# distributed-lab/bp-pp

Hardware: AMD Instinct MI355X
Metric: u64 range-proof batch verifies/sec (higher is better)
Workload: dtype u32; 1 GPU; batch verify ONE fixed batch of 1048576 independent u64 range proofs (BASELINE configs[2]; all resident on one GPU), exact per-proof mode, shared generators, inputs resident in HBM, 1/1024 proofs corrupted, one 4-byte reject-count all-reduce per step; proofs_per_gpu=1048576, fb_window_bits=523, fb_window_bits_hi=0, fb_hi_bases=0, fb_window_bits_chosen_by=the library, from the HBM free at context creation, label=u64 range proof, parallelism=single, full=False

## Files before the change

bp_pp_amd/csrc/straus_core.h:

```cpp
#pragma once
#include "verify_ws.h"

namespace bppp {

struct straus_scalar { u32 kp[8]; u32 top; };
HD void straus_recode(straus_scalar& r, const sc& k) {
    u64 c = 0;
#pragma unroll
    for (int i = 0; i < 8; i++) { c += (u64)k.v[i] + 0x88888888u; r.kp[i] = (u32)c; c >>= 32; }
    r.top = (u32)c;
}
HD void straus_build_table(pt_slot* tbl, const apt& P) {
    pt cur;
    pt_set_identity(cur);
    tbl[0].p = cur;
    pt_from_affine(cur, P);
    tbl[1].p = cur;
    const bool pid = apt_is_identity(P);
#pragma nounroll
    for (int e = 2; e <= 8; e++) {
        pt src = tbl[(e & 1) ? e - 1 : e / 2].p;
        pt d;
        if (e & 1) pt_madd(d, src, P, pid);
        else pt_dbl(d, src);
        pt_normalize(d);
        tbl[e].p = d;
    }
}
HD void straus_msm(pt& out, const pt_slot* tbl, const straus_scalar* rs, int m) {
    pt acc;
    pt_set_identity(acc);
#pragma nounroll
    for (int j = 0; j < m; j++) {
        pt q = tbl[j * BPPP_STRAUS_ENTRIES + (rs[j].top ? 1 : 0)].p;
        pt_add(acc, acc, q);
    }
#pragma nounroll
    for (int i = 63; i >= 0; i--) {
#pragma nounroll
        for (int d = 0; d < 4; d++) pt_dbl(acc, acc);
#pragma nounroll
        for (int j = 0; j < m; j++) {
            u32 limb = 0;
#pragma unroll
            for (int l = 0; l < 8; l++) limb = (l == (i >> 3)) ? rs[j].kp[l] : limb;
            int dg = (int)((limb >> ((i & 7) * 4)) & 15) - 8;
            int mag = dg < 0 ? -dg : dg;
            pt q = tbl[j * BPPP_STRAUS_ENTRIES + mag].p;
            fe ny;
            fe_neg_m<1>(ny, q.Y);
            fe_cmov(q.Y, dg < 0, ny);
            pt_add(acc, acc, q);
        }
    }
    out = acc;
}

struct glv_split { u32 k1[5], k2[5]; bool neg1, neg2; };
HD void glv_round_shift384(sc& c, const sc& k, const u32 g[8]) {
    u32 t[16];
    mul256(t, k.v, g);
    u32 cy = (t[11] >> 31) & 1u;
#pragma unroll
    for (int i = 0; i < 4; i++) c.v[i] = addc(t[12 + i], 0u, cy);
#pragma unroll
    for (int i = 4; i < 8; i++) c.v[i] = 0;
}
HD bool glv_abs(u32 out[5], const sc& r) {
    bool neg = ((r.v[5] | r.v[6] | r.v[7]) != 0) | (r.v[4] > 1u);
    sc m;
    sc_neg(m, r);
#pragma unroll
    for (int i = 0; i < 5; i++) out[i] = neg ? m.v[i] : r.v[i];
    return neg;
}
HD void glv_decompose(glv_split& out, const sc& k) {
    const u32 G1[8] = {0x45DBB031u, 0xE893209Au, 0x71E8CA7Fu, 0x3DAA8A14u, 0x9284EB15u, 0xE86C90E4u, 0xA7D46BCDu, 0x3086D221u};
    const u32 G2[8] = {0x8AC47F71u, 0x1571B4AEu, 0x9DF506C6u, 0x221208ACu, 0x0ABFE4C4u, 0x6F547FA9u, 0x010E8828u, 0xE4437ED6u};
    const sc MB1 = {{0x0ABFE4C3u, 0x6F547FA9u, 0x010E8828u, 0xE4437ED6u, 0x00000000u, 0x00000000u, 0x00000000u, 0x00000000u}};
    const sc MB2 = {{0x3DB1562Cu, 0xD765CDA8u, 0x0774346Du, 0x8A280AC5u, 0xFFFFFFFEu, 0xFFFFFFFFu, 0xFFFFFFFFu, 0xFFFFFFFFu}};
    const sc LAM = {{0x1B23BD72u, 0xDF02967Cu, 0x20816678u, 0x122E22EAu, 0x8812645Au, 0xA5261C02u, 0xC05C30E0u, 0x5363AD4Cu}};
    sc c1, c2, r1, r2, t;
    glv_round_shift384(c1, k, G1);
    glv_round_shift384(c2, k, G2);
    sc_mul(c1, c1, MB1);
    sc_mul(c2, c2, MB2);
    sc_add(r2, c1, c2);
    sc_mul(t, r2, LAM);
    sc_sub(r1, k, t);
    out.neg1 = glv_abs(out.k1, r1);
    out.neg2 = glv_abs(out.k2, r2);
    u32 c = 0;
#pragma unroll
    for (int i = 0; i < 5; i++) out.k1[i] = addc(out.k1[i], i < 4 ? 0x88888888u : 0x8u, c);
    c = 0;
#pragma unroll
    for (int i = 0; i < 5; i++) out.k2[i] = addc(out.k2[i], i < 4 ? 0x88888888u : 0x8u, c);
}
HD u32 limb5_at(const u32 v[5], int idx) {
    u32 r = 0;
#pragma unroll
    for (int l = 0; l < 5; l++) r = (l == idx) ? v[l] : r;
    return r;
}
HD void straus_msm_glv(pt& out, const pt_slot* tbl, const glv_split* sp, int m) {
    const u32 BETA_W[8] = {0x719501EEu, 0xC1396C28u, 0x12F58995u, 0x9CF04975u, 0xAC3434E9u, 0x6E64479Eu, 0x657C0710u, 0x7AE96A2Bu};
    fe BETA;
    fe_from_w8(BETA, BETA_W);
    pt acc;
    pt_set_identity(acc);
#pragma nounroll
    for (int i = 32; i >= 0; i--) {
        if (i != 32) {
#pragma nounroll
            for (int d = 0; d < 4; d++) pt_dbl(acc, acc);
        }
#pragma nounroll
        for (int j = 0; j < m; j++) {
#pragma nounroll
            for (int h = 0; h < 2; h++) {
                const u32* kp = h ? sp[j].k2 : sp[j].k1;
                bool sneg = h ? sp[j].neg2 : sp[j].neg1;
                int dg = (int)((limb5_at(kp, i >> 3) >> ((i & 7) * 4)) & 15) - 8;
                int mag = dg < 0 ? -dg : dg;
                pt q = tbl[j * BPPP_STRAUS_ENTRIES + mag].p;
                fe bx, ny;
                fe_mul(bx, q.X, BETA);
                fe_cmov(q.X, h != 0, bx);
                fe_neg_m<1>(ny, q.Y);
                fe_cmov(q.Y, (dg < 0) != sneg, ny);
                pt_add(acc, acc, q);
            }
        }
    }
    out = acc;
}

#define BPPP_VPOINTS 13
#define BPPP_ATAB_PER_PROOF (BPPP_VPOINTS * 16)
HD void ws_st_fe(u32* base, size_t N, size_t t, int slot, const fe& a) {
#pragma unroll
    for (int i = 0; i < 10; i++) base[(size_t)(slot * 10 + i) * N + t] = a.v[i];
}
HD void ws_ld_fe(fe& a, const u32* base, size_t N, size_t t, int slot, int mag) {
#pragma unroll
    for (int i = 0; i < 10; i++) a.v[i] = base[(size_t)(slot * 10 + i) * N + t];
    FE_SETMAG(a, mag);
    (void)mag;
}
template <int G>
HD void fe_batch_inv_lane(const u32* in, u32* out, size_t N, size_t i) {
    const size_t L = (N + G - 1) / G;
    fe z[G], pre[G], run, inv, one;
    bool zero[G];
    fe_set_u32(one, 1);
    run = one;
#pragma unroll
    for (int j = 0; j < G; j++) {
        const size_t t = i + (size_t)j * L;
        z[j] = one;
        zero[j] = true;
        if (t < N) {
            ws_ld_fe(z[j], in, N, t, 0, 2);
            zero[j] = fe_is_zero(z[j]);
            if (zero[j]) z[j] = one;
        }
        pre[j] = run;
        fe_mul(run, run, z[j]);
    }
    fe_inv(inv, run);
#pragma unroll
    for (int j = G - 1; j >= 0; j--) {
        const size_t t = i + (size_t)j * L;
        fe o;
        fe_mul(o, inv, pre[j]);
        fe_mul(inv, inv, z[j]);
        if (zero[j]) fe_set_u32(o, 0);
        if (t < N) ws_st_fe(out, N, t, 0, o);
    }
}
HD void glv_beta(fe& b) {
    const u32 BETA_W[8] = {0x719501EEu, 0xC1396C28u, 0x12F58995u, 0x9CF04975u, 0xAC3434E9u, 0x6E64479Eu, 0x657C0710u, 0x7AE96A2Bu};
    fe_from_w8(b, BETA_W);
}
struct atab_ref {
    apt_packed* p;
    size_t s;
    HD apt_packed& operator[](int i) const { return p[(size_t)i * s]; }
    HD atab_ref operator+(int k) const { atab_ref r = {p + (size_t)k * s, s}; return r; }
};
HD atab_ref atab_of(apt_packed* atab, size_t N, size_t t, int entries_per_instance = 13 * 16) {
    (void)entries_per_instance;
    atab_ref r = {atab + t, N};
    return r;
}
HD void atab_store(atab_ref tb, int e, const apt& a, const fe& beta, bool identity) {
    apt_packed k;
    fe_to_w8(k.x, a.x);
    fe_to_w8(k.y, a.y);
    if (identity) {
#pragma unroll
        for (int i = 0; i < 8; i++) k.x[i] = k.y[i] = 0;
    }
    tb[e - 1] = k;
    (void)beta;
}
#define BPPP_TSCR_FE (5 * BPPP_VPOINTS)
struct aff_src { fe x, y; };
HD void aff_ld(aff_src& r, atab_ref tb, int e) {
    const apt_packed k = tb[e - 1];
    fe_from_w8(r.x, k.x);
    fe_from_w8(r.y, k.y);
}
HD void aff_den_dbl(fe& d, const aff_src& a, bool pid, const fe& one) { fe_add(d, a.y, a.y); fe_cmov(d, pid, one); }
HD void aff_den_add(fe& d, const aff_src& a, const aff_src& b, bool pid, const fe& one) { fe_sub_m<1>(d, a.x, b.x); fe_cmov(d, pid, one); }
HD void aff_dbl(apt& r, const aff_src& a, const fe& dinv) {
    fe num, lam, t;
    fe_sqr(num, a.x);
    fe_mul_small(num, num, 3);
    fe_mul(lam, num, dinv);
    fe_sqr(r.x, lam);
    fe_add(t, a.x, a.x);
    fe_sub_m<2>(r.x, r.x, t);
    fe_sub_m<4>(t, a.x, r.x);
    fe_mul(t, lam, t);
    fe_sub_m<1>(r.y, t, a.y);
}
HD void aff_add(apt& r, const aff_src& a, const aff_src& b, const fe& dinv) {
    fe num, lam, t;
    fe_sub_m<1>(num, a.y, b.y);
    fe_mul(lam, num, dinv);
    fe_sqr(r.x, lam);
    fe_sub_m<1>(r.x, r.x, a.x);
    fe_sub_m<1>(r.x, r.x, b.x);
    fe_sub_m<5>(t, a.x, r.x);
    fe_mul(t, lam, t);
    fe_sub_m<1>(r.y, t, a.y);
}
HD void aff_take(aff_src& r, const apt& a) {
    fe_mul_small(r.x, a.x, 1);
    fe_mul_small(r.y, a.y, 1);
}
HD void aff_push(u32* tscr, size_t N, size_t t, int slot, fe& run, const fe& den) {
    ws_st_fe(tscr, N, t, slot, run);
    fe_mul(run, run, den);
}
HD void aff_pop(fe& dinv, const u32* tscr, size_t N, size_t t, int slot, fe& inv, const fe& den) {
    fe pre;
    ws_ld_fe(pre, tscr, N, t, slot, 1);
    fe_mul(dinv, inv, pre);
    fe_mul(inv, inv, den);
}
HD void aff_push_block(u32* tscr, size_t N, size_t t, int slot, fe& run, const fe& block_product) {
    ws_st_fe(tscr, N, t, slot, run);
    fe_mul(run, run, block_product);
}
HD void aff_pop_block(fe di[4], const fe d[4], const u32* tscr, size_t N, size_t t, int slot, fe& inv) {
    fe t01, t23, B, pre, q;
    fe_mul(t01, d[0], d[1]);
    fe_mul(t23, d[2], d[3]);
    fe_mul(B, t01, t23);
    ws_ld_fe(pre, tscr, N, t, slot, 1);
    fe_mul(q, inv, pre);
    fe_mul(inv, inv, B);
    fe_mul(B, q, t23);
    fe_mul(q, q, t01);
    fe_mul(di[0], B, d[1]);
    fe_mul(di[1], B, d[0]);
    fe_mul(di[2], q, d[3]);
    fe_mul(di[3], q, d[2]);
}
#define BPPP_TSCR_PER_POINT 5
HD void affine_tables_pass_a(const atab_ref tab, u32* tscr, const u32* pts, size_t N, size_t t, const int NP, fe& run) {
    const int L2 = NP, L4 = 3 * NP;
    (void)L2; (void)L4;
    fe beta, one, d, dinv;
    fe_set_u32(one, 1);
    glv_beta(beta);
    (void)d; (void)dinv;
    fe_set_u32(run, 1);
#pragma nounroll
    for (int p = 0; p < NP; p++) {
        apt P;
        ws_ld_apt(P, pts, N, t, p);
        const bool pid = apt_is_identity(P);
        atab_store(tab + p * 16, 1, P, beta, pid);
        aff_src a = {P.x, P.y};
        aff_den_dbl(d, a, pid, one);
        aff_push(tscr, N, t, p, run, d);
    }
}
HD void affine_tables_pass_b(const atab_ref tab, u32* tscr, const u32* pts, size_t N, size_t t, const int NP, fe inv, fe& run) {
    const int L2 = NP, L4 = 3 * NP;
    (void)L2; (void)L4;
    fe beta, one, d, dinv;
    fe_set_u32(one, 1);
    glv_beta(beta);
    (void)d; (void)dinv;
    fe_set_u32(run, 1);
#pragma nounroll
    for (int p = NP - 1; p >= 0; p--) {
        apt P;
        ws_ld_apt(P, pts, N, t, p);
        const bool pid = apt_is_identity(P);
        aff_src a = {P.x, P.y};
        aff_den_dbl(d, a, pid, one);
        aff_pop(dinv, tscr, N, t, p, inv, d);
        apt P2;
        aff_dbl(P2, a, dinv);
        atab_store(tab + p * 16, 2, P2, beta, pid);
        aff_src a2;
        aff_take(a2, P2);
        const int q = L2 + (NP - 1 - p) * 2;
        aff_den_add(d, a2, a, pid, one);
        aff_push(tscr, N, t, q, run, d);
        aff_den_dbl(d, a2, pid, one);
        aff_push(tscr, N, t, q + 1, run, d);
    }
}
HD void affine_tables_pass_c(const atab_ref tab, u32* tscr, const u32* pts, size_t N, size_t t, const int NP, fe inv, fe& run) {
    const int L2 = NP, L4 = 3 * NP;
    (void)L2; (void)L4;
    fe beta, one, d, dinv;
    fe_set_u32(one, 1);
    glv_beta(beta);
    (void)d; (void)dinv;
    fe_set_u32(run, 1);
#pragma nounroll
    for (int p = 0; p < NP; p++) {
        const atab_ref tb = tab + p * 16;
        aff_src a, a2;
        aff_ld(a, tb, 1);
        aff_ld(a2, tb, 2);
        const bool pid = fe_is_zero(a.x) & fe_is_zero(a.y);
        const int q = L2 + (NP - 1 - p) * 2;
        apt P3, P4;
        aff_den_dbl(d, a2, pid, one);
        aff_pop(dinv, tscr, N, t, q + 1, inv, d);
        aff_dbl(P4, a2, dinv);
        aff_den_add(d, a2, a, pid, one);
        aff_pop(dinv, tscr, N, t, q, inv, d);
        aff_add(P3, a2, a, dinv);
        atab_store(tb, 3, P3, beta, pid);
        atab_store(tb, 4, P4, beta, pid);
        aff_src a3, a4;
        aff_take(a3, P3);
        aff_take(a4, P4);
        fe bp;
        aff_den_add(bp, a4, a, pid, one);
        aff_den_dbl(d, a3, pid, one);
        fe_mul(bp, bp, d);
        aff_den_add(d, a4, a3, pid, one);
        fe_mul(bp, bp, d);
        aff_den_dbl(d, a4, pid, one);
        fe_mul(bp, bp, d);
        aff_push_block(tscr, N, t, p, run, bp);
    }
}
HD void affine_tables_pass_d(const atab_ref tab, u32* tscr, const u32* pts, size_t N, size_t t, const int NP, fe inv, fe& run) {
    const int L2 = NP, L4 = 3 * NP;
    (void)L2; (void)L4;
    fe beta, one, d, dinv;
    fe_set_u32(one, 1);
    glv_beta(beta);
    (void)d; (void)dinv;
    fe_set_u32(run, 1);
#pragma nounroll
    for (int p = NP - 1; p >= 0; p--) {
        const atab_ref tb = tab + p * 16;
        aff_src a, a3, a4;
        aff_ld(a, tb, 1);
        aff_ld(a3, tb, 3);
        aff_ld(a4, tb, 4);
        const bool pid = fe_is_zero(a.x) & fe_is_zero(a.y);
        fe dd[4], di[4];
        aff_den_add(dd[0], a4, a, pid, one);
        aff_den_dbl(dd[1], a3, pid, one);
        aff_den_add(dd[2], a4, a3, pid, one);
        aff_den_dbl(dd[3], a4, pid, one);
        aff_pop_block(di, dd, tscr, N, t, p, inv);
        apt R;
        fe x8, bo, be;
        aff_src ax;
        aff_dbl(R, a4, di[3]);
        atab_store(tb, 8, R, beta, pid);
        aff_take(ax, R);
        x8 = ax.x;
        aff_den_dbl(be, ax, pid, one);
        fe_sub_m<1>(bo, x8, a.x);  fe_cmov(bo, pid, one);
        fe_sub_m<1>(d, x8, a3.x);  fe_cmov(d, pid, one);  fe_mul(bo, bo, d);
        aff_add(R, a4, a3, di[2]);
        atab_store(tb, 7, R, beta, pid);
        aff_take(ax, R);
        fe_sub_m<1>(d, x8, ax.x);  fe_cmov(d, pid, one);  fe_mul(bo, bo, d);
        aff_den_dbl(d, ax, pid, one);                     fe_mul(be, be, d);
        aff_dbl(R, a3, di[1]);
        atab_store(tb, 6, R, beta, pid);
        aff_take(ax, R);
        aff_den_dbl(d, ax, pid, one);                     fe_mul(be, be, d);
        aff_add(R, a4, a, di[0]);
        atab_store(tb, 5, R, beta, pid);
        aff_take(ax, R);
        fe_sub_m<1>(d, x8, ax.x);  fe_cmov(d, pid, one);  fe_mul(bo, bo, d);
        aff_den_dbl(d, ax, pid, one);                     fe_mul(be, be, d);
        aff_push_block(tscr, N, t, L4 + 2 * p, run, bo);
        aff_push_block(tscr, N, t, L4 + 2 * p + 1, run, be);
    }
}
HD void affine_tables_pass_e(const atab_ref tab, u32* tscr, const u32* pts, size_t N, size_t t, const int NP, fe inv) {
    const int L2 = NP, L4 = 3 * NP;
    (void)L2; (void)L4;
    fe beta, one, d, dinv;
    fe_set_u32(one, 1);
    glv_beta(beta);
    (void)d; (void)dinv;
#pragma nounroll
    for (int p = 0; p < NP; p++) {
        const atab_ref tb = tab + p * 16;
        aff_src a5, a6, a7, a8;
        aff_ld(a5, tb, 5);
        aff_ld(a8, tb, 8);
        const bool pid = fe_is_zero(a8.x) & fe_is_zero(a8.y);
        fe dd[4], di[4];
        apt R;
        aff_ld(a6, tb, 6);
        aff_ld(a7, tb, 7);
        aff_den_dbl(dd[0], a5, pid, one);
        aff_den_dbl(dd[1], a6, pid, one);
        aff_den_dbl(dd[2], a7, pid, one);
        aff_den_dbl(dd[3], a8, pid, one);
        aff_pop_block(di, dd, tscr, N, t, L4 + 2 * p + 1, inv);
        aff_dbl(R, a5, di[0]);  atab_store(tb, 10, R, beta, pid);
        aff_dbl(R, a6, di[1]);  atab_store(tb, 12, R, beta, pid);
        aff_dbl(R, a7, di[2]);  atab_store(tb, 14, R, beta, pid);
        aff_dbl(R, a8, di[3]);  atab_store(tb, 16, R, beta, pid);
        aff_src a, a3;
        aff_ld(a, tb, 1);
        aff_ld(a3, tb, 3);
        aff_den_add(dd[0], a8, a, pid, one);
        aff_den_add(dd[1], a8, a3, pid, one);
        aff_den_add(dd[2], a8, a5, pid, one);
        aff_den_add(dd[3], a8, a7, pid, one);
        aff_pop_block(di, dd, tscr, N, t, L4 + 2 * p, inv);
        aff_add(R, a8, a, di[0]);   atab_store(tb, 9, R, beta, pid);
        aff_add(R, a8, a3, di[1]);  atab_store(tb, 11, R, beta, pid);
        aff_add(R, a8, a5, di[2]);  atab_store(tb, 13, R, beta, pid);
        aff_add(R, a8, a7, di[3]);  atab_store(tb, 15, R, beta, pid);
    }
}
HD void affine_tables_build(const atab_ref tab, u32* tscr, const u32* pts, size_t N, size_t t, const int NP) {
    fe run, inv;
    affine_tables_pass_a(tab, tscr, pts, N, t, NP, run);
    fe_inv(inv, run);
    affine_tables_pass_b(tab, tscr, pts, N, t, NP, inv, run);
    fe_inv(inv, run);
    affine_tables_pass_c(tab, tscr, pts, N, t, NP, inv, run);
    fe_inv(inv, run);
    affine_tables_pass_d(tab, tscr, pts, N, t, NP, inv, run);
    fe_inv(inv, run);
    affine_tables_pass_e(tab, tscr, pts, N, t, NP, inv);
}
template <int PASS>
HD void verify_tables_pass(const VerifyWs& ws, size_t t) {
    const atab_ref tab = atab_of(ws.atab, ws.N, t);
    fe run, inv;
    if constexpr (PASS > 0) ws_ld_fe(inv, ws.zinv, ws.N, t, 0, 1);
    if constexpr (PASS == 0) affine_tables_pass_a(tab, ws.tscr, ws.pts, ws.N, t, BPPP_VPOINTS, run);
    if constexpr (PASS == 1) affine_tables_pass_b(tab, ws.tscr, ws.pts, ws.N, t, BPPP_VPOINTS, inv, run);
    if constexpr (PASS == 2) affine_tables_pass_c(tab, ws.tscr, ws.pts, ws.N, t, BPPP_VPOINTS, inv, run);
    if constexpr (PASS == 3) affine_tables_pass_d(tab, ws.tscr, ws.pts, ws.N, t, BPPP_VPOINTS, inv, run);
    if constexpr (PASS == 4) affine_tables_pass_e(tab, ws.tscr, ws.pts, ws.N, t, BPPP_VPOINTS, inv);
    if constexpr (PASS < 4) ws_st_fe(ws.zinv, ws.N, t, 0, run);
}
HD void verify_tables(const VerifyWs& ws, size_t t) {
    BPPP_STAMP(t, 16);
    affine_tables_build(atab_of(ws.atab, ws.N, t), ws.tscr, ws.pts, ws.N, t, BPPP_VPOINTS);
    BPPP_STAMP(t, 19);
}
HD void verify_tables_own(const VerifyWs& ws, size_t t) {
    const size_t N = ws.N;
    u32* tp = ws.fsc + (size_t)(17 * 8) * N;
    const uint8_t* pv = ws.commitments + 64 * t;
    const uint8_t* pp = ws.proofs + (size_t)BPPP_U64_PROOF_BYTES * t;
    apt V, Pr;
    bool ok = apt_from_xy64(V, pv);
#pragma nounroll
    for (int i = 0; i < 12; i++) {
        apt Q;
        ok &= apt_from_xy64(Q, pp + 64 * i);
        ws_st_apt(tp, N, t, i, Q);
    }
    ok &= apt_from_xy64(Pr, pp + 64 * 12);
    sc l0;
    ok &= sc_from_be(l0, pp + 832);
    ok &= sc_from_be(l0, pp + 864);
    ok &= sc_from_be(l0, pp + 896);
    if (!ok) {
        apt zero;
        fe_set_u32(zero.x, 0);
        fe_set_u32(zero.y, 0);
        V = zero;
        Pr = zero;
#pragma nounroll
        for (int i = 0; i < 12; i++) ws_st_apt(tp, N, t, i, zero);
    }
    apt Vr;
    {
        pt s;
        pt_from_affine(s, V);
        pt_madd(s, s, Pr, apt_is_identity(Pr));
        pt_to_affine(Vr, s);
    }
    ws_st_apt(tp, N, t, 12, Vr);
    affine_tables_build(atab_of(ws.atab, ws.N, t), ws.tscr, tp, N, t, BPPP_VPOINTS);
}
#define BPPP_SPLIT_PARTS_MAX 4
HD int split_begin(int parts, int part) {
    if (parts == 1) return part == 0 ? 0 : 26;
    if (parts == 2) return part == 0 ? 0 : part == 1 ? 13 : 26;
    return part == 0 ? 0 : part == 1 ? 7 : part == 2 ? 14 : part == 3 ? 20 : 26;
}
HD void affine_table_one(atab_ref tb, const apt& Pin, int pre_doublings) {
    fe beta;
    glv_beta(beta);
    apt P = Pin;
    const bool pid = apt_is_identity(Pin);
    if (pre_doublings) {
        ptj a;
        bool e0 = true;
        ptj_init(a);
        ptj_madd(a, e0, P, false);
#pragma nounroll
        for (int d = 0; d < pre_doublings; d++) ptj_dbl(a);
        fe zi, zi2;
        fe_inv(zi, a.Z);
        fe_sqr(zi2, zi);
        fe_mul(P.x, a.X, zi2);
        fe_mul(zi2, zi2, zi);
        fe_mul(P.y, a.Y, zi2);
    }
    atab_store(tb, 1, P, beta, pid);
    ptj T;
    bool empty = true;
    ptj_init(T);
    ptj_madd(T, empty, P, false);
    ptj_dbl(T);
    fe jx[15], jy[15], jz[15], pre[15];
#pragma nounroll
    for (int k = 0; k < 15; k++) {
        if (k) ptj_madd(T, empty, P, false);
        jx[k] = T.X; jy[k] = T.Y; jz[k] = T.Z;
        if (k) fe_mul(pre[k], pre[k - 1], T.Z);
        else fe_mul_small(pre[0], T.Z, 1);
    }
    fe inv;
    fe_inv(inv, pre[14]);
#pragma nounroll
    for (int k = 14; k >= 0; k--) {
        fe zi, zi2;
        if (k) { fe_mul(zi, inv, pre[k - 1]); fe_mul(inv, inv, jz[k]); }
        else zi = inv;
        apt R;
        fe_sqr(zi2, zi);
        fe_mul(R.x, jx[k], zi2);
        fe_mul(zi2, zi2, zi);
        fe_mul(R.y, jy[k], zi2);
        atab_store(tb, k + 2, R, beta, pid);
    }
}
HD void verify_table_source(apt& P, const VerifyWs& ws, size_t t, int p) {
    const uint8_t* pv = ws.commitments + 64 * t;
    const uint8_t* pp = ws.proofs + (size_t)BPPP_U64_PROOF_BYTES * t;
    apt V, Pr, Q;
    fe_set_u32(P.x, 0);
    fe_set_u32(P.y, 0);
    bool ok = apt_from_xy64(V, pv);
#pragma nounroll
    for (int i = 0; i < 12; i++) {
        ok &= apt_from_xy64(Q, pp + 64 * i);
        if (i == p) P = Q;
    }
    ok &= apt_from_xy64(Pr, pp + 64 * 12);
    sc k;
    ok &= sc_from_be(k, pp + 832);
    ok &= sc_from_be(k, pp + 864);
    ok &= sc_from_be(k, pp + 896);
    if (p == 12 && ok) {
        pt s;
        pt_from_affine(s, V);
        pt_madd(s, s, Pr, apt_is_identity(Pr));
        pt_to_affine(P, s);
    }
    if (!ok) { fe_set_u32(P.x, 0); fe_set_u32(P.y, 0); }
}
HD void verify_table_one(const VerifyWs& ws, size_t t, int p, int h, int parts, bool from_bytes = false) {
    apt P;
    if (from_bytes) verify_table_source(P, ws, t, p);
    else ws_ld_apt(P, ws.pts, ws.N, t, p);
    affine_table_one(atab_of(ws.atab, ws.N, t) + (h * BPPP_VPOINTS + p) * 16, P, 5 * split_begin(parts, h));
}
template <int M>
struct glv_words {
    u32 w[2 * M][5];
    bool neg[2 * M];
};
#define BPPP_STRAUS_WINDOWS 26
HD void glv_recode5(u32 out[5], const u32 k4[5]) {
    const u32 D[5] = {0x987FB988u, 0x7FB987FBu, 0xB987FB98u, 0x87FB987Fu, 0xFFFFFFF9u};
    u32 c = 0;
#pragma unroll
    for (int i = 0; i < 5; i++) out[i] = addc(k4[i], D[i], c);
}
template <int M>
HD void glv_words_set(glv_words<M>& g, int j, const glv_split& sp) {
    glv_recode5(g.w[2 * j], sp.k1);
    glv_recode5(g.w[2 * j + 1], sp.k2);
    g.neg[2 * j] = sp.neg1;
    g.neg[2 * j + 1] = sp.neg2;
}
template <int M>
HD u64 glv_window_digits(const glv_words<M>& g, int i) {
    const int b = 5 * i, l = b >> 5, sh = b & 31;
    u64 pk = 0;
#pragma unroll
    for (int st = 0; st < 2 * M; st++) {
        u32 lo = 0, hi = 0;
#pragma unroll
        for (int q = 0; q < 5; q++) {
            lo = (q == l) ? g.w[st][q] : lo;
            hi = (q == l + 1) ? g.w[st][q] : hi;
        }
        const u32 v = (u32)(((((u64)hi) << 32) | lo) >> sh) & 31u;
        pk |= (u64)v << (5 * st);
    }
    return pk;
}
template <int M>
HD void glv_digit_of(const glv_words<M>& g, u64 pk, int r, int& mag, bool& neg) {
    bool sneg = false;
#pragma unroll
    for (int st = 0; st < 2 * M; st++) sneg = (st == r) ? g.neg[st] : sneg;
    const int dg = (int)((pk >> (5 * r)) & 31u) - 16;
    mag = dg < 0 ? -dg : dg;
    neg = (dg < 0) != sneg;
}
HD void straus_pace(bool pace, int window) {
#if defined(__HIP_DEVICE_COMPILE__)
    if (!pace) return;
    if (window >= 13) __builtin_amdgcn_s_setprio(3);
    else if (window >= 6) __builtin_amdgcn_s_setprio(2);
    else if (window >= 3) __builtin_amdgcn_s_setprio(1);
    else __builtin_amdgcn_s_setprio(0);
#else
    (void)pace; (void)window;
#endif
}
template <int M>
HD bool straus_affine_fast(pt& out, atab_ref tab, const int* pidx, const glv_words<M>& g, bool pace = false) {
    const int total = BPPP_STRAUS_WINDOWS * 2 * M;
    fe beta;
    glv_beta(beta);
    straus_pace(pace, BPPP_STRAUS_WINDOWS - 1);
    ptj acc;
    ptj_init(acc);
    bool empty = true;
    apt_packed cur_e, nxt_e;
    int cur_mag, nxt_mag;
    bool cur_neg, nxt_neg;
    u64 pk_cur = glv_window_digits<M>(g, BPPP_STRAUS_WINDOWS - 1), pk_nxt = glv_window_digits<M>(g, BPPP_STRAUS_WINDOWS - 2);
    glv_digit_of<M>(g, pk_cur, 0, cur_mag, cur_neg);
    cur_e = tab[pidx[0] * 16 + (cur_mag ? cur_mag - 1 : 0)];
    int r = 0, i = BPPP_STRAUS_WINDOWS - 1;
#pragma nounroll
    for (int s = 0; s < total; s++) {
        int rn = r + 1, in = i;
        if (rn == 2 * M) { rn = 0; in = i - 1; }
        if (in < 0) { rn = r; in = i; }
        glv_digit_of<M>(g, in == i ? pk_cur : pk_nxt, rn, nxt_mag, nxt_neg);
        int pn = 0;
#pragma unroll
        for (int j = 0; j < M; j++) pn = (j == (rn >> 1)) ? pidx[j] : pn;
        nxt_e = tab[pn * 16 + (nxt_mag ? nxt_mag - 1 : 0)];
        if (r == 0 && s != 0) {
            straus_pace(pace, i);
#pragma nounroll
            for (int d = 0; d < 5; d++) ptj_dbl(acc);
        }
        apt e;
        bool id;
        apt_unpack(e, id, cur_e);
        if (r & 1) fe_mul(e.x, e.x, beta);
        fe ny;
        fe_neg_m<1>(ny, e.y);
        fe_cmov(e.y, cur_neg, ny);
        ptj_madd(acc, empty, e, (cur_mag == 0) | id);
        cur_e = nxt_e;
        cur_mag = nxt_mag;
        cur_neg = nxt_neg;
        if (in != i) { pk_cur = pk_nxt; pk_nxt = glv_window_digits<M>(g, in > 0 ? in - 1 : 0); }
        r = rn;
        i = in;
    }
    const bool exceptional = !empty && fe_is_zero(acc.Z);
    ptj_to_pt(out, acc, empty);
    return !exceptional;
}
template <int M>
HD void straus_affine_complete(pt& out, atab_ref tab, const int* pidx, const glv_words<M>& g) {
    fe beta;
    glv_beta(beta);
    pt acc;
    pt_set_identity(acc);
#pragma nounroll
    for (int i = BPPP_STRAUS_WINDOWS - 1; i >= 0; i--) {
        if (i != BPPP_STRAUS_WINDOWS - 1) {
#pragma nounroll
            for (int d = 0; d < 5; d++) pt_dbl(acc, acc);
        }
        const u64 pk = glv_window_digits<M>(g, i);
#pragma nounroll
        for (int r = 0; r < 2 * M; r++) {
            int mag, pn = 0;
            bool neg, id;
            glv_digit_of<M>(g, pk, r, mag, neg);
#pragma unroll
            for (int j = 0; j < M; j++) pn = (j == (r >> 1)) ? pidx[j] : pn;
            apt e;
            apt_unpack(e, id, tab[pn * 16 + (mag ? mag - 1 : 0)]);
            if (r & 1) fe_mul(e.x, e.x, beta);
            fe ny;
            fe_neg_m<1>(ny, e.y);
            fe_cmov(e.y, neg, ny);
            pt_madd(acc, acc, e, (mag == 0) | id);
        }
    }
    out = acc;
}
template <int M>
HD void straus_affine(pt& out, atab_ref tab, const int* pidx, const glv_words<M>& g, bool pace = false) {
    if (!straus_affine_fast<M>(out, tab, pidx, g, pace)) {
        glv_words<M> gc = g;
        int pc[M];
#pragma unroll
        for (int j = 0; j < M; j++) pc[j] = pidx[j];
        pt o;
        straus_affine_complete<M>(o, tab, pc, gc);
        out = o;
    }
}

template <int M>
HD bool straus_split_lane(pt& part, atab_ref tab, const int* pidx, const glv_words<M>& g, int q, int parts, int stride = BPPP_VPOINTS) {
    fe beta;
    glv_beta(beta);
    const bool have = q < 2 * M * parts;
    const int h = have ? q / (2 * M) : 0, r = have ? q - 2 * M * h : 0;
    u32 w[5];
    bool sneg = false;
    int pn = 0;
#pragma unroll
    for (int l = 0; l < 5; l++) w[l] = 0;
#pragma unroll
    for (int st = 0; st < 2 * M; st++) {
#pragma unroll
        for (int l = 0; l < 5; l++) w[l] = (st == r) ? g.w[st][l] : w[l];
        sneg = (st == r) ? g.neg[st] : sneg;
        pn = (st == r) ? pidx[st >> 1] : pn;
    }
    const bool img = (r & 1) != 0;
    const int base = (pn + stride * h) * 16, w0 = split_begin(parts, h), nw = split_begin(parts, h + 1) - w0;
    auto digit = [&](int i, int& mag, bool& neg) {
        const int b = 5 * i, l = b >> 5, sh = b & 31;
        u32 lo = 0, hi = 0;
#pragma unroll
        for (int k = 0; k < 5; k++) { lo = (k == l) ? w[k] : lo; hi = (k == l + 1) ? w[k] : hi; }
        const int dg = (int)((u32)(((((u64)hi) << 32) | lo) >> sh) & 31u) - 16;
        mag = dg < 0 ? -dg : dg;
        neg = (dg < 0) != sneg;
    };
    ptj acc;
    ptj_init(acc);
    bool empty = true;
    int cur_mag, nxt_mag;
    bool cur_neg, nxt_neg;
    apt_packed cur_e, nxt_e;
    digit(w0 + nw - 1, cur_mag, cur_neg);
    cur_e = tab[base + (cur_mag ? cur_mag - 1 : 0)];
#pragma nounroll
    for (int i = nw - 1; i >= 0; i--) {
        digit(w0 + (i > 0 ? i - 1 : 0), nxt_mag, nxt_neg);
        nxt_e = tab[base + (nxt_mag ? nxt_mag - 1 : 0)];
        if (i != nw - 1) {
#pragma nounroll
            for (int d = 0; d < 5; d++) ptj_dbl(acc);
        }
        apt e;
        bool id;
        apt_unpack(e, id, cur_e);
        fe bx, ny;
        fe_mul(bx, e.x, beta);
        fe_cmov(e.x, img, bx);
        fe_neg_m<1>(ny, e.y);
        fe_cmov(e.y, cur_neg, ny);
        ptj_madd(acc, empty, e, (cur_mag == 0) | id | !have);
        cur_e = nxt_e;
        cur_mag = nxt_mag;
        cur_neg = nxt_neg;
    }
    const bool exceptional = !empty && fe_is_zero(acc.Z);
    ptj_to_pt(part, acc, empty);
    return !exceptional;
}
#if defined(__HIPCC__)
template <int M, int G = 4>
__device__ __forceinline__ void straus_affine_g4(pt& out, atab_ref tab, const int* pidx, const glv_words<M>& g, int q) {
    constexpr int NS = (2 * M + G - 1) / G;
    fe beta;
    glv_beta(beta);
    u32 w[NS][5];
    bool sneg[NS], img[NS], have[NS];
    int pn[NS];
#pragma unroll
    for (int j = 0; j < NS; j++) {
        const int r = q + G * j;
        have[j] = r < 2 * M;
        sneg[j] = false;
        pn[j] = 0;
#pragma unroll
        for (int l = 0; l < 5; l++) w[j][l] = 0;
#pragma unroll
        for (int st = 0; st < 2 * M; st++) {
#pragma unroll
            for (int l = 0; l < 5; l++) w[j][l] = (st == r) ? g.w[st][l] : w[j][l];
            sneg[j] = (st == r) ? g.neg[st] : sneg[j];
            pn[j] = (st == r) ? pidx[st >> 1] : pn[j];
        }
        img[j] = (r & 1) != 0;
    }
    auto digit = [&](const u32 (&ww)[5], bool sn, int i, int& mag, bool& neg) {
        const int b = 5 * i, l = b >> 5, sh = b & 31;
        u32 lo = 0, hi = 0;
#pragma unroll
        for (int k = 0; k < 5; k++) { lo = (k == l) ? ww[k] : lo; hi = (k == l + 1) ? ww[k] : hi; }
        const int dg = (int)((u32)(((((u64)hi) << 32) | lo) >> sh) & 31u) - 16;
        mag = dg < 0 ? -dg : dg;
        neg = (dg < 0) != sn;
    };
    ptj acc;
    ptj_init(acc);
    bool empty = true;
    int cur_mag[NS], nxt_mag[NS];
    bool cur_neg[NS], nxt_neg[NS];
    apt_packed cur_e[NS], nxt_e[NS];
#pragma unroll
    for (int j = 0; j < NS; j++) {
        digit(w[j], sneg[j], BPPP_STRAUS_WINDOWS - 1, cur_mag[j], cur_neg[j]);
        cur_e[j] = tab[pn[j] * 16 + (cur_mag[j] ? cur_mag[j] - 1 : 0)];
    }
#pragma nounroll
    for (int i = BPPP_STRAUS_WINDOWS - 1; i >= 0; i--) {
#pragma unroll
        for (int j = 0; j < NS; j++) {
            digit(w[j], sneg[j], i > 0 ? i - 1 : 0, nxt_mag[j], nxt_neg[j]);
            nxt_e[j] = tab[pn[j] * 16 + (nxt_mag[j] ? nxt_mag[j] - 1 : 0)];
        }
        if (i != BPPP_STRAUS_WINDOWS - 1) {
#pragma nounroll
            for (int d = 0; d < 5; d++) ptj_dbl(acc);
        }
#pragma unroll
        for (int j = 0; j < NS; j++) {
            apt e;
            bool id;
            apt_unpack(e, id, cur_e[j]);
            fe bx, ny;
            fe_mul(bx, e.x, beta);
            fe_cmov(e.x, img[j], bx);
            fe_neg_m<1>(ny, e.y);
            fe_cmov(e.y, cur_neg[j], ny);
            ptj_madd(acc, empty, e, (cur_mag[j] == 0) | id | !have[j]);
            cur_e[j] = nxt_e[j];
            cur_mag[j] = nxt_mag[j];
            cur_neg[j] = nxt_neg[j];
        }
    }
    int bad = (!empty && fe_is_zero(acc.Z)) ? 1 : 0;
#pragma unroll
    for (int m = 1; m < G; m <<= 1) bad |= __shfl_xor(bad, m, 64);
    if (bad) {
        straus_affine_complete<M>(out, tab, pidx, g);
        return;
    }
    pt part;
    ptj_to_pt(part, acc, empty);
    lane_group_sum<G>(part);
    out = part;
}
template <int M, int G, int PARTS>
__device__ __forceinline__ void straus_affine_split(pt& out, atab_ref tab, const int* pidx, const glv_words<M>& g, int q, int stride = BPPP_VPOINTS) {
    static_assert(2 * M * PARTS <= G, "a lane per part of a stream");
    pt part;
    int bad = straus_split_lane<M>(part, tab, pidx, g, q, PARTS, stride) ? 0 : 1;
#pragma unroll
    for (int m = 1; m < G; m <<= 1) bad |= __shfl_xor(bad, m, 64);
    if (bad) {
        straus_affine_complete<M>(out, tab, pidx, g);
        return;
    }
    lane_group_sum<G>(part);
    out = part;
}
#endif


}
```

Before: 7.010 million verifies/s.

## Restructure affine table build with shared-inverse add/sub pairs and fewer scratch slots

Reorganizes the batched-inversion affine precomputation of the 16-entry point tables. Entries are now derived as P±Q pairs that share one denominator inverse (computing 5 and 3, 9 and 7, 10 and 6, and 14, 15 via subtraction). This cuts the number of denominators per point and shrinks scratch from 5 to 3 field elements per point. Passes a and b are merged into one pass and a sixth pass is added, so the number of launches stays the same. The cost is an extra sequential inversion stage and a more intricate dependency order, which makes correctness harder to check.

```diff
diff --git a/bp_pp_amd/csrc/straus_core.h b/bp_pp_amd/csrc/straus_core.h
--- a/bp_pp_amd/csrc/straus_core.h
+++ b/bp_pp_amd/csrc/straus_core.h
@@ -205,12 +205,16 @@
     tb[e - 1] = k;
     (void)beta;
 }
-#define BPPP_TSCR_FE (5 * BPPP_VPOINTS)
+#define BPPP_TSCR_FE (BPPP_TSCR_PER_POINT * BPPP_VPOINTS)
+#define BPPP_TSCR_PER_POINT 3
 struct aff_src { fe x, y; };
 HD void aff_ld(aff_src& r, atab_ref tb, int e) {
     const apt_packed k = tb[e - 1];
     fe_from_w8(r.x, k.x);
     fe_from_w8(r.y, k.y);
+}
+HD void aff_ld_x(fe& x, atab_ref tb, int e) {
+    fe_from_w8(x, tb[e - 1].x);
 }
 HD void aff_den_dbl(fe& d, const aff_src& a, bool pid, const fe& one) { fe_add(d, a.y, a.y); fe_cmov(d, pid, one); }
 HD void aff_den_add(fe& d, const aff_src& a, const aff_src& b, bool pid, const fe& one) { fe_sub_m<1>(d, a.x, b.x); fe_cmov(d, pid, one); }
@@ -236,6 +240,35 @@
     fe_sub_m<5>(t, a.x, r.x);
     fe_mul(t, lam, t);
     fe_sub_m<1>(r.y, t, a.y);
+}
+HD void aff_sub(apt& r, const aff_src& a, const aff_src& b, const fe& dinv) {
+    fe num, lam, t;
+    fe_add(num, a.y, b.y);
+    fe_mul(lam, num, dinv);
+    fe_sqr(r.x, lam);
+    fe_sub_m<1>(r.x, r.x, a.x);
+    fe_sub_m<1>(r.x, r.x, b.x);
+    fe_sub_m<5>(t, a.x, r.x);
+    fe_mul(t, lam, t);
+    fe_sub_m<1>(r.y, t, a.y);
+}
+HD void aff_add_sub(apt& rp, apt& rm, const aff_src& a, const aff_src& b, const fe& dinv) {
+    fe num, lam, t, sx;
+    fe_add(sx, a.x, b.x);
+    fe_sub_m<1>(num, a.y, b.y);
+    fe_mul(lam, num, dinv);
+    fe_sqr(rp.x, lam);
+    fe_sub_m<2>(rp.x, rp.x, sx);
+    fe_sub_m<4>(t, a.x, rp.x);
+    fe_mul(t, lam, t);
+    fe_sub_m<1>(rp.y, t, a.y);
+    fe_add(num, a.y, b.y);
+    fe_mul(lam, num, dinv);
+    fe_sqr(rm.x, lam);
+    fe_sub_m<2>(rm.x, rm.x, sx);
+    fe_sub_m<4>(t, a.x, rm.x);
+    fe_mul(t, lam, t);
+    fe_sub_m<1>(rm.y, t, a.y);
 }
 HD void aff_take(aff_src& r, const apt& a) {
     fe_mul_small(r.x, a.x, 1);
@@ -270,10 +303,18 @@
     fe_mul(di[2], q, d[3]);
     fe_mul(di[3], q, d[2]);
 }
-#define BPPP_TSCR_PER_POINT 5
+HD void aff_pop_pair(fe di[2], const fe d[2], const u32* tscr, size_t N, size_t t, int slot, fe& inv) {
+    fe B, pre, q;
+    fe_mul(B, d[0], d[1]);
+    ws_ld_fe(pre, tscr, N, t, slot, 1);
+    fe_mul(q, inv, pre);
+    fe_mul(inv, inv, B);
+    fe_mul(di[0], q, d[1]);
+    fe_mul(di[1], q, d[0]);
+}
 HD void affine_tables_pass_a(const atab_ref tab, u32* tscr, const u32* pts, size_t N, size_t t, const int NP, fe& run) {
-    const int L2 = NP, L4 = 3 * NP;
-    (void)L2; (void)L4;
+    const int L2 = NP;
+    (void)L2;
     fe beta, one, d, dinv;
     fe_set_u32(one, 1);
     glv_beta(beta);
@@ -291,8 +332,8 @@
     }
 }
 HD void affine_tables_pass_b(const atab_ref tab, u32* tscr, const u32* pts, size_t N, size_t t, const int NP, fe inv, fe& run) {
-    const int L2 = NP, L4 = 3 * NP;
-    (void)L2; (void)L4;
+    const int L2 = NP;
+    (void)L2;
     fe beta, one, d, dinv;
     fe_set_u32(one, 1);
     glv_beta(beta);
@@ -311,16 +352,13 @@
         atab_store(tab + p * 16, 2, P2, beta, pid);
         aff_src a2;
         aff_take(a2, P2);
-        const int q = L2 + (NP - 1 - p) * 2;
-        aff_den_add(d, a2, a, pid, one);
-        aff_push(tscr, N, t, q, run, d);
         aff_den_dbl(d, a2, pid, one);
-        aff_push(tscr, N, t, q + 1, run, d);
+        aff_push(tscr, N, t, L2 + 2 * p, run, d);
     }
 }
 HD void affine_tables_pass_c(const atab_ref tab, u32* tscr, const u32* pts, size_t N, size_t t, const int NP, fe inv, fe& run) {
-    const int L2 = NP, L4 = 3 * NP;
-    (void)L2; (void)L4;
+    const int L2 = NP;
+    (void)L2;
     fe beta, one, d, dinv;
     fe_set_u32(one, 1);
     glv_beta(beta);
@@ -333,33 +371,23 @@
         aff_ld(a, tb, 1);
         aff_ld(a2, tb, 2);
         const bool pid = fe_is_zero(a.x) & fe_is_zero(a.y);
-        const int q = L2 + (NP - 1 - p) * 2;
-        apt P3, P4;
+        apt P4;
         aff_den_dbl(d, a2, pid, one);
-        aff_pop(dinv, tscr, N, t, q + 1, inv, d);
+        aff_pop(dinv, tscr, N, t, L2 + 2 * p, inv, d);
         aff_dbl(P4, a2, dinv);
-        aff_den_add(d, a2, a, pid, one);
-        aff_pop(dinv, tscr, N, t, q, inv, d);
-        aff_add(P3, a2, a, dinv);
-        atab_store(tb, 3, P3, beta, pid);
         atab_store(tb, 4, P4, beta, pid);
-        aff_src a3, a4;
-        aff_take(a3, P3);
+        aff_src a4;
         aff_take(a4, P4);
         fe bp;
-        aff_den_add(bp, a4, a, pid, one);
-        aff_den_dbl(d, a3, pid, one);
-        fe_mul(bp, bp, d);
-        aff_den_add(d, a4, a3, pid, one);
-        fe_mul(bp, bp, d);
-        aff_den_dbl(d, a4, pid, one);
+        aff_den_dbl(bp, a4, pid, one);
+        aff_den_add(d, a4, a, pid, one);
         fe_mul(bp, bp, d);
         aff_push_block(tscr, N, t, p, run, bp);
     }
 }
 HD void affine_tables_pass_d(const atab_ref tab, u32* tscr, const u32* pts, size_t N, size_t t, const int NP, fe inv, fe& run) {
-    const int L2 = NP, L4 = 3 * NP;
-    (void)L2; (void)L4;
+    const int L2 = NP;
+    (void)L2;
     fe beta, one, d, dinv;
     fe_set_u32(one, 1);
     glv_beta(beta);
@@ -368,108 +396,133 @@
 #pragma nounroll
     for (int p = NP - 1; p >= 0; p--) {
         const atab_ref tb = tab + p * 16;
-        aff_src a, a3, a4;
+        aff_src a, a2, a4;
         aff_ld(a, tb, 1);
-        aff_ld(a3, tb, 3);
         aff_ld(a4, tb, 4);
         const bool pid = fe_is_zero(a.x) & fe_is_zero(a.y);
-        fe dd[4], di[4];
-        aff_den_add(dd[0], a4, a, pid, one);
-        aff_den_dbl(dd[1], a3, pid, one);
-        aff_den_add(dd[2], a4, a3, pid, one);
-        aff_den_dbl(dd[3], a4, pid, one);
-        aff_pop_block(di, dd, tscr, N, t, p, inv);
-        apt R;
-        fe x8, bo, be;
-        aff_src ax;
-        aff_dbl(R, a4, di[3]);
+        fe dd[2], di[2];
+        aff_den_dbl(dd[0], a4, pid, one);
+        aff_den_add(dd[1], a4, a, pid, one);
+        aff_pop_pair(di, dd, tscr, N, t, p, inv);
+        apt R, Rm;
+        fe bj, b8;
+        aff_src a8, ax;
+        aff_dbl(R, a4, di[0]);
         atab_store(tb, 8, R, beta, pid);
+        aff_take(a8, R);
+        aff_den_dbl(b8, a8, pid, one);
+        aff_den_add(d, a8, a4, pid, one);                 fe_mul(b8, b8, d);
+        aff_den_add(bj, a8, a, pid, one);
+        aff_ld_x(a2.x, tb, 2);
+        aff_den_add(d, a8, a2, pid, one);                 fe_mul(bj, bj, d);
+        aff_add_sub(R, Rm, a4, a, di[1]);
+        atab_store(tb, 5, R, beta, pid);
+        atab_store(tb, 3, Rm, beta, pid);
+        aff_take(ax, Rm);
+        aff_den_add(d, a8, ax, pid, one);                 fe_mul(bj, bj, d);
         aff_take(ax, R);
-        x8 = ax.x;
-        aff_den_dbl(be, ax, pid, one);
-        fe_sub_m<1>(bo, x8, a.x);  fe_cmov(bo, pid, one);
-        fe_sub_m<1>(d, x8, a3.x);  fe_cmov(d, pid, one);  fe_mul(bo, bo, d);
-        aff_add(R, a4, a3, di[2]);
-        atab_store(tb, 7, R, beta, pid);
-        aff_take(ax, R);
-        fe_sub_m<1>(d, x8, ax.x);  fe_cmov(d, pid, one);  fe_mul(bo, bo, d);
-        aff_den_dbl(d, ax, pid, one);                     fe_mul(be, be, d);
-        aff_dbl(R, a3, di[1]);
-        atab_store(tb, 6, R, beta, pid);
-        aff_take(ax, R);
-        aff_den_dbl(d, ax, pid, one);                     fe_mul(be, be, d);
-        aff_add(R, a4, a, di[0]);
-        atab_store(tb, 5, R, beta, pid);
-        aff_take(ax, R);
-        fe_sub_m<1>(d, x8, ax.x);  fe_cmov(d, pid, one);  fe_mul(bo, bo, d);
-        aff_den_dbl(d, ax, pid, one);                     fe_mul(be, be, d);
-        aff_push_block(tscr, N, t, L4 + 2 * p, run, bo);
-        aff_push_block(tscr, N, t, L4 + 2 * p + 1, run, be);
-    }
-}
-HD void affine_tables_pass_e(const atab_ref tab, u32* tscr, const u32* pts, size_t N, size_t t, const int NP, fe inv) {
-    const int L2 = NP, L4 = 3 * NP;
-    (void)L2; (void)L4;
+        aff_den_add(d, a8, ax, pid, one);                 fe_mul(bj, bj, d);
+        aff_push_block(tscr, N, t, L2 + 2 * p, run, bj);
+        aff_push_block(tscr, N, t, L2 + 2 * p + 1, run, b8);
+    }
+}
+HD void affine_tables_pass_e(const atab_ref tab, u32* tscr, const u32* pts, size_t N, size_t t, const int NP, fe inv, fe& run) {
+    const int L2 = NP;
+    (void)L2;
     fe beta, one, d, dinv;
     fe_set_u32(one, 1);
     glv_beta(beta);
     (void)d; (void)dinv;
+    fe_set_u32(run, 1);
 #pragma nounroll
     for (int p = 0; p < NP; p++) {
         const atab_ref tb = tab + p * 16;
-        aff_src a5, a6, a7, a8;
-        aff_ld(a5, tb, 5);
+        aff_src a8, ax;
         aff_ld(a8, tb, 8);
         const bool pid = fe_is_zero(a8.x) & fe_is_zero(a8.y);
-        fe dd[4], di[4];
+        fe dd[4], di[4], bp;
+        apt R, Rm;
+        aff_ld(ax, tb, 4);
+        aff_den_dbl(dd[0], a8, pid, one);
+        aff_den_add(dd[1], a8, ax, pid, one);
+        aff_pop_pair(di, dd, tscr, N, t, L2 + 2 * p + 1, inv);
+        aff_add(R, a8, ax, di[1]);  atab_store(tb, 12, R, beta, pid);
+        aff_dbl(R, a8, di[0]);      atab_store(tb, 16, R, beta, pid);
+        fe x16, x1, x2;
+        fe_mul_small(x16, R.x, 1);
+        aff_ld_x(x1, tb, 1);
+        aff_ld_x(x2, tb, 2);
+        fe_sub_m<1>(bp, x16, x2);  fe_cmov(bp, pid, one);
+        fe_sub_m<1>(d, x16, x1);   fe_cmov(d, pid, one);
+        fe_mul(bp, bp, d);
+        aff_push_block(tscr, N, t, p, run, bp);
+        fe_sub_m<1>(dd[0], a8.x, x1);  fe_cmov(dd[0], pid, one);
+        fe_sub_m<1>(dd[1], a8.x, x2);  fe_cmov(dd[1], pid, one);
+        aff_ld_x(x1, tb, 3);
+        aff_ld_x(x2, tb, 5);
+        fe_sub_m<1>(dd[2], a8.x, x1);  fe_cmov(dd[2], pid, one);
+        fe_sub_m<1>(dd[3], a8.x, x2);  fe_cmov(dd[3], pid, one);
+        aff_pop_block(di, dd, tscr, N, t, L2 + 2 * p, inv);
+        aff_ld(ax, tb, 1);
+        aff_add_sub(R, Rm, a8, ax, di[0]);  atab_store(tb, 9, R, beta, pid);   atab_store(tb, 7, Rm, beta, pid);
+        aff_ld(ax, tb, 2);
+        aff_add_sub(R, Rm, a8, ax, di[1]);  atab_store(tb, 10, R, beta, pid);  atab_store(tb, 6, Rm, beta, pid);
+        aff_ld(ax, tb, 3);
+        aff_add(R, a8, ax, di[2]);          atab_store(tb, 11, R, beta, pid);
+        aff_ld(ax, tb, 5);
+        aff_add(R, a8, ax, di[3]);          atab_store(tb, 13, R, beta, pid);
+    }
+}
+HD void affine_tables_pass_f(const atab_ref tab, u32* tscr, const u32* pts, size_t N, size_t t, const int NP, fe inv) {
+    fe beta, one;
+    fe_set_u32(one, 1);
+    glv_beta(beta);
+    (void)pts;
+#pragma nounroll
+    for (int p = NP - 1; p >= 0; p--) {
+        const atab_ref tb = tab + p * 16;
+        aff_src a, a2, a16;
+        aff_ld(a16, tb, 16);
+        aff_ld(a2, tb, 2);
+        aff_ld(a, tb, 1);
+        const bool pid = fe_is_zero(a16.x) & fe_is_zero(a16.y);
+        fe dd[2], di[2];
         apt R;
-        aff_ld(a6, tb, 6);
-        aff_ld(a7, tb, 7);
-        aff_den_dbl(dd[0], a5, pid, one);
-        aff_den_dbl(dd[1], a6, pid, one);
-        aff_den_dbl(dd[2], a7, pid, one);
-        aff_den_dbl(dd[3], a8, pid, one);
-        aff_pop_block(di, dd, tscr, N, t, L4 + 2 * p + 1, inv);
-        aff_dbl(R, a5, di[0]);  atab_store(tb, 10, R, beta, pid);
-        aff_dbl(R, a6, di[1]);  atab_store(tb, 12, R, beta, pid);
-        aff_dbl(R, a7, di[2]);  atab_store(tb, 14, R, beta, pid);
-        aff_dbl(R, a8, di[3]);  atab_store(tb, 16, R, beta, pid);
-        aff_src a, a3;
-        aff_ld(a, tb, 1);
-        aff_ld(a3, tb, 3);
-        aff_den_add(dd[0], a8, a, pid, one);
-        aff_den_add(dd[1], a8, a3, pid, one);
-        aff_den_add(dd[2], a8, a5, pid, one);
-        aff_den_add(dd[3], a8, a7, pid, one);
-        aff_pop_block(di, dd, tscr, N, t, L4 + 2 * p, inv);
-        aff_add(R, a8, a, di[0]);   atab_store(tb, 9, R, beta, pid);
-        aff_add(R, a8, a3, di[1]);  atab_store(tb, 11, R, beta, pid);
-        aff_add(R, a8, a5, di[2]);  atab_store(tb, 13, R, beta, pid);
-        aff_add(R, a8, a7, di[3]);  atab_store(tb, 15, R, beta, pid);
-    }
-}
-HD void affine_tables_build(const atab_ref tab, u32* tscr, const u32* pts, size_t N, size_t t, const int NP) {
-    fe run, inv;
+        aff_den_add(dd[0], a16, a2, pid, one);
+        aff_den_add(dd[1], a16, a, pid, one);
+        aff_pop_pair(di, dd, tscr, N, t, p, inv);
+        aff_sub(R, a16, a2, di[0]);  atab_store(tb, 14, R, beta, pid);
+        aff_sub(R, a16, a, di[1]);   atab_store(tb, 15, R, beta, pid);
+    }
+}
+HD void affine_tables_pass_ab(const atab_ref tab, u32* tscr, const u32* pts, size_t N, size_t t, const int NP, fe& run) {
+    fe inv;
     affine_tables_pass_a(tab, tscr, pts, N, t, NP, run);
     fe_inv(inv, run);
     affine_tables_pass_b(tab, tscr, pts, N, t, NP, inv, run);
+}
+HD void affine_tables_build(const atab_ref tab, u32* tscr, const u32* pts, size_t N, size_t t, const int NP) {
+    fe run, inv;
+    affine_tables_pass_ab(tab, tscr, pts, N, t, NP, run);
     fe_inv(inv, run);
     affine_tables_pass_c(tab, tscr, pts, N, t, NP, inv, run);
     fe_inv(inv, run);
     affine_tables_pass_d(tab, tscr, pts, N, t, NP, inv, run);
     fe_inv(inv, run);
-    affine_tables_pass_e(tab, tscr, pts, N, t, NP, inv);
+    affine_tables_pass_e(tab, tscr, pts, N, t, NP, inv, run);
+    fe_inv(inv, run);
+    affine_tables_pass_f(tab, tscr, pts, N, t, NP, inv);
 }
 template <int PASS>
 HD void verify_tables_pass(const VerifyWs& ws, size_t t) {
     const atab_ref tab = atab_of(ws.atab, ws.N, t);
     fe run, inv;
     if constexpr (PASS > 0) ws_ld_fe(inv, ws.zinv, ws.N, t, 0, 1);
-    if constexpr (PASS == 0) affine_tables_pass_a(tab, ws.tscr, ws.pts, ws.N, t, BPPP_VPOINTS, run);
-    if constexpr (PASS == 1) affine_tables_pass_b(tab, ws.tscr, ws.pts, ws.N, t, BPPP_VPOINTS, inv, run);
-    if constexpr (PASS == 2) affine_tables_pass_c(tab, ws.tscr, ws.pts, ws.N, t, BPPP_VPOINTS, inv, run);
-    if constexpr (PASS == 3) affine_tables_pass_d(tab, ws.tscr, ws.pts, ws.N, t, BPPP_VPOINTS, inv, run);
-    if constexpr (PASS == 4) affine_tables_pass_e(tab, ws.tscr, ws.pts, ws.N, t, BPPP_VPOINTS, inv);
+    if constexpr (PASS == 0) affine_tables_pass_ab(tab, ws.tscr, ws.pts, ws.N, t, BPPP_VPOINTS, run);
+    if constexpr (PASS == 1) affine_tables_pass_c(tab, ws.tscr, ws.pts, ws.N, t, BPPP_VPOINTS, inv, run);
+    if constexpr (PASS == 2) affine_tables_pass_d(tab, ws.tscr, ws.pts, ws.N, t, BPPP_VPOINTS, inv, run);
+    if constexpr (PASS == 3) affine_tables_pass_e(tab, ws.tscr, ws.pts, ws.N, t, BPPP_VPOINTS, inv, run);
+    if constexpr (PASS == 4) affine_tables_pass_f(tab, ws.tscr, ws.pts, ws.N, t, BPPP_VPOINTS, inv);
     if constexpr (PASS < 4) ws_st_fe(ws.zinv, ws.N, t, 0, run);
 }
 HD void verify_tables(const VerifyWs& ws, size_t t) {
```

New measurement: 6.961 million verifies/s. About the same (-0.7%).
